# getzlab/rnaseqc

Hardware: AMD Instinct MI355X
Metric: reads/sec whole-node (100 M-read synthetic BAM, GENCODE GTF) at 1/2/4/8 GPU -- `value`: the hot path over the records resident in HBM (the bench contract's definition of value); `whole_node.value`: the same job from the BAM file to the reports (CLI `Average Reads/Sec` window), checked against `value (higher is better)
Workload: dtype i32/u64 counters, f64 exon fractions

## Files before the change

rnaseqc_amd/csrc/rsqc_api.cpp:

```cpp
#include "rsqc_ctx.h"
#include "rsqc_index.h"

namespace rsqc {

int fail(rsqc_ctx *c, int code, const std::string &msg) {
    if (c) { c->last_error = msg; }
    return code;
}
int dev_alloc(rsqc_ctx *c, DevBuf &b, size_t bytes, bool zero) {
    if (bytes == 0) bytes = 16;
    bytes = (bytes + 15) & ~(size_t)15;
    if (b.bytes < bytes) {
        b.release();
        HIP_TRY(c, hipMalloc(&b.p, bytes));
        b.bytes = bytes;
    }
    if (zero) HIP_TRY(c, hipMemsetAsync(b.p, 0, b.bytes, c->stream));
    return 0;
}
bool dev_reserve(DevBuf &b, size_t bytes) {
    if (b.bytes >= bytes) return true;
    b.release();
    if (hipMalloc(&b.p, bytes) != hipSuccess) { (void)hipGetLastError(); b.p = nullptr; return false; }
    b.bytes = bytes;
    return true;
}
bool host_reserve(HostBuf &b, size_t bytes) {
    if (b.bytes >= bytes) return true;
    b.release();
    if (hipHostMalloc(&b.p, bytes, hipHostMallocDefault) != hipSuccess) { (void)hipGetLastError(); b.p = nullptr; return false; }
    b.bytes = bytes;
    return true;
}

static int zero_accumulators(rsqc_ctx *c) {
    launch_reset(c->stream, c->d_arena.p, c->arena_bytes, c->d_cov.p, c->d_cov.bytes, (uint32_t *)((char *)c->d_arena.p + c->off_misc + 36));
    HIP_TRY(c, hipGetLastError());
    for (auto &pb : c->pair_pool) pb.used = false;
    c->pairs_in_flight.clear();
    c->pair_arena.used = c->frag_arena.used = c->gc_arena.used = 0;
    for (auto &fb : c->frag_pool) fb.used = false;
    c->frags_in_flight.clear();
    c->h_fsize.clear(); c->h_fcount.clear();
    c->frag_remaining = c->have_bed ? c->params.fragment_samples : 0;
    for (auto &gb : c->gc_pool) gb.used = false;
    c->gcs_in_flight.clear();
    if (c->have_ref) {
        HIP_TRY(c, hipMemsetAsync(c->d_gc_bins.p, 0, (RSQC_GC_BINS + 1) * 8, c->stream));
        c->h_gc.assign(RSQC_GC_BINS + 1, 0);
    }
    c->finalized = false;
    c->next_record_base = 0; c->name_mode = -1; c->have_ranges = false; c->have_composed_rl = false;
    c->batch_file_index.clear(); c->batch_records.clear();
    c->h_rl_offset.clear(); c->h_rl_span.clear(); c->h_rl_state.clear();
    c->h_sample_file.clear(); c->h_sample_size.clear(); c->frag_kept = 0;
    c->sticky = 0;
    return 0;
}

// ... 57 lines not shown
        if (D.ev_copy) (void)hipEventDestroy(D.ev_copy);
        if (D.copy_stream) (void)hipStreamDestroy(D.copy_stream);
        for (auto &e : D.pe) if (e) (void)hipEventDestroy(e);
    }
    sort_drop(c);
    markdup_drop(c);
    junction_drop(c, true);
    track_drop(c, true);
    genebody_drop(c, true);
    tin_drop(c, true);
    cycle_drop(c, true);
    mismatch_drop(c, true);
    for (auto &b : c->parked) b.release();
    free_sort_scratch(c->gc_scratch); free_sort_scratch(c->frag_scratch);
    c->d_ref_bits.release(); c->d_ref_off.release(); c->d_ref_len.release(); c->d_gc_bins.release(); c->d_exon_gc.release();
    DevBuf *all[] = {&c->d_arena, &c->d_cov, &c->d_ovf_index, &c->d_tiles, &c->d_defer, &c->d_ei_rank, &c->d_table, &c->d_tab_off, &c->d_tab_cap};
    if (c->h_arena) (void)hipHostFree(c->h_arena);
    if (c->h_rl_raw) (void)hipHostFree(c->h_rl_raw);
    if (c->stream2) (void)hipStreamDestroy(c->stream2);
    if (c->stream3) (void)hipStreamDestroy(c->stream3);
    if (c->stream4) (void)hipStreamDestroy(c->stream4);
    if (c->ev_join3) (void)hipEventDestroy(c->ev_join3);
    if (c->ev_join4) (void)hipEventDestroy(c->ev_join4);
    if (c->ev_fork) (void)hipEventDestroy(c->ev_fork);
    if (c->ev_retired) (void)hipEventDestroy(c->ev_retired);
    if (c->ev_join) (void)hipEventDestroy(c->ev_join);
    for (auto *b : all) b->release();
    for (auto &pr : c->k1_events) { (void)hipEventDestroy(pr.first); (void)hipEventDestroy(pr.second); }
    for (auto &pr : c->long_events) (void)hipEventDestroy(pr.second);
    for (auto e : c->event_pool) (void)hipEventDestroy(e);
    (void)hipStreamDestroy(c->stream);
    delete c;
}

int rsqc_set_annotation(rsqc_ctx *c, const rsqc_annotation *a, const uint8_t *owned_contig) {
    if (!c || !a) return RSQC_ERR_ARG;
    if (c->have_ann) return fail(c, RSQC_ERR_ARG, "annotation already set");
    HIP_TRY(c, hipSetDevice(c->device));
    const int nc = a->n_contigs, G = a->n_genes, L = a->n_genes_listed, E = a->n_exons;
    c->n_ref = a->n_ref; c->n_contigs = nc; c->n_genes = G; c->n_listed = L; c->n_exons = E;
    HostIndex hx;
    {
        std::string err;
        int brc = hx.build(a, owned_contig, err);
        if (brc) return fail(c, brc, err);
    }
    const uint64_t run = hx.cov_entries;
// ... 47 lines not shown
#undef UPV
#undef UPA
    const size_t n_u64 = (size_t)G * 3 + RSQC_N_COUNTERS;
    const size_t Lz = (size_t)std::max(L, 1), Ez = (size_t)std::max(E, 1);
    auto pad8 = [](size_t x) { return (x + 7) & ~(size_t)7; };
    size_t at = 0;
    c->off_u64 = at; at += n_u64 * 8;
    c->off_bias3 = at; at += Lz * 8;
    c->off_bias5 = at; at += Lz * 8;
    c->off_exon = at; at += Ez * 8;
    c->off_gmean = at; at += Lz * 8;
    c->off_gstd = at; at += Lz * 8;
    c->off_gcv = at; at += Lz * 8;
    c->off_ecv = at; at += Ez * 8;
    c->off_gvalid = at; at += pad8(Lz);
    c->off_ecvv = at; at += pad8(Ez);
    c->off_ehit = at; at += pad8(Ez);
    at = (at + 15) & ~(size_t)15;
    c->off_misc = at; at += 64;
    c->arena_bytes = at;
    if ((rc = dev_alloc(c, c->d_arena, at, false))) return rc;
    HIP_TRY(c, hipHostMalloc((void **)&c->h_arena, at, hipHostMallocDefault));
    if ((rc = dev_alloc(c, c->d_cov, (size_t)(run + 64) * 4, false))) return rc;
    const uint32_t ovf_cap = 1u << 20;
    if ((rc = dev_alloc(c, c->d_ovf_index, (size_t)ovf_cap * 8, false))) return rc;
    for (hipStream_t *s : {&c->stream2, &c->stream3, &c->stream4})
        if (!*s) HIP_TRY(c, hipStreamCreateWithPriority(s, hipStreamNonBlocking, c->prio_side));
    for (hipEvent_t *e : {&c->ev_join3, &c->ev_join4, &c->ev_fork, &c->ev_join, &c->ev_retired})
        if (!*e) HIP_TRY(c, hipEventCreateWithFlags(e, hipEventDisableTiming));
    char *A = (char *)c->d_arena.p;
    DevAccum &acc = c->acc;
    acc.gene_reads = (unsigned long long *)(A + c->off_u64);
    acc.gene_unique = acc.gene_reads + G;
    acc.gene_frag = acc.gene_unique + G;
    acc.counters = acc.gene_frag + G;
    acc.exon_acc = (double *)(A + c->off_exon);
    acc.cov_diff = (uint32_t *)c->d_cov.p;
    acc.ovf_count = (uint32_t *)(A + c->off_misc);
    acc.read_length = (int32_t *)(A + c->off_misc + 8);
    acc.error = (int *)(A + c->off_misc + 16);
    acc.rl_stats = (uint32_t *)(A + c->off_misc + 32);
    acc.defer_total = (uint32_t *)(A + c->off_misc + 48);
    acc.ovf_index = (uint64_t *)c->d_ovf_index.p; acc.ovf_cap = ovf_cap;
    c->have_ann = true;
    if ((rc = zero_accumulators(c))) return rc;
    HIP_TRY(c, hipStreamSynchronize(c->stream));
    c->last_error = hx.warning;
    c->n_exons_outside_gene = hx.n_exons_outside_gene;
    return RSQC_OK;
}

// ... 126 lines not shown
    for (auto &pb : c->pair_pool) pb.used = false;
    for (auto &fb : c->frag_pool) fb.used = false;
    for (auto &gb : c->gc_pool) gb.used = false;
    c->pairs_in_flight.clear(); c->frags_in_flight.clear(); c->gcs_in_flight.clear();
    for (Arena *a : {&c->pair_arena, &c->frag_arena, &c->gc_arena}) {
        for (int k = 0; k < a->n_col; ++k) a->col[k].release();
        a->used = a->cap = 0;
    }
    for (auto &b : c->ann_bufs) b.release();
    c->ann_bufs.clear();
    for (DevBuf *b : {&c->d_arena, &c->d_cov, &c->d_ei_rank, &c->d_ovf_index, &c->d_table, &c->d_tab_off, &c->d_tab_cap,
                      &c->d_ref_bits, &c->d_ref_off, &c->d_ref_len, &c->d_gc_bins, &c->d_exon_gc,
                      &c->d_rl_summary}) b->release();
    if (c->h_arena) { (void)hipHostFree(c->h_arena); c->h_arena = nullptr; }
    c->arena_bytes = 0;
    c->dann = DevAnnotation{}; c->dref = DevReference{};
    uint32_t *const tile_span = c->acc.tile_span;
    c->acc = DevAccum{}; c->acc.tile_span = tile_span;
    c->d_ge_off = c->d_ge_row = c->d_gene_cov_off = c->d_gene_coding = c->d_gene_order = nullptr;
    c->d_gene_flags = c->d_gene_owned = nullptr;
    c->n_ref = c->n_contigs = c->n_genes = c->n_listed = c->n_exons = 0;
    c->k3_large = c->k3_medium = c->k3_xlarge = c->k3_le6144 = c->k3_le3072 = c->k3_le2048 = c->k3_le1024 = 0;
    c->cov_entries = 0; c->n_exons_outside_gene = 0;
    std::vector<uint32_t>().swap(c->exon_row_id);
    std::vector<double>().swap(c->h_exon_gc);
    c->h_gc.clear();
    c->have_ann = c->have_bed = c->have_ref = false;
    free_sort_scratch(c->gc_scratch); free_sort_scratch(c->frag_scratch);
    c->h_fsize.clear(); c->h_fcount.clear(); c->frag_remaining = 0; c->frag_kept = 0;
    c->finalized = false; c->early_copied = false;
    c->next_record_base = 0; c->name_mode = -1; c->have_ranges = false; c->have_composed_rl = false;
    c->batch_file_index.clear(); c->batch_records.clear();
    c->h_rl_offset.clear(); c->h_rl_span.clear(); c->h_rl_state.clear();
    c->h_sample_file.clear(); c->h_sample_size.clear();
    c->results = rsqc_results{};
    c->sticky = 0;
    c->last_error.clear();
    return RSQC_OK;
}

void *rsqc_host_alloc(size_t bytes) {
    void *p = nullptr;
    if (hipHostMalloc(&p, bytes ? bytes : 16, hipHostMallocDefault) != hipSuccess) { (void)hipGetLastError(); return nullptr; }
    return p;
}
void rsqc_host_free(void *p) { if (p) (void)hipHostFree(p); }
// ... 49 lines not shown
```

rnaseqc_amd/csrc/rsqc_ctx.h:

```cpp
#pragma once
#include <algorithm>
#include <chrono>
#include <cstdio>
#include <cstdlib>
#include <cstring>
#include <string>
#include <vector>

#include "rsqc_device.h"
#include "rsqc_decode.h"
#include "rsqc_sam.h"

#if defined(RSQC_K1_PROF) || defined(RSQC_DIAG_KNOBS)
#define RSQC_DIAG(name) getenv(name)
namespace rsqc {
inline void host_trace(const char *what) {
    static const bool on = getenv("RSQC_HOST_TRACE") != nullptr;
    if (!on) return;
    static std::chrono::steady_clock::time_point last = std::chrono::steady_clock::now();
    const auto now = std::chrono::steady_clock::now();
    fprintf(stderr, "[host] %-28s +%8.1f us\n", what, std::chrono::duration<double, std::micro>(now - last).count());
    last = now;
}
}
// ... 192 lines not shown
    bool have_ann = false;
    int32_t n_ref = 0, n_contigs = 0, n_genes = 0, n_listed = 0, n_exons = 0;
    std::vector<uint32_t> exon_row_id;
    std::vector<DevBuf> ann_bufs;
    DevAnnotation dann{};
    DevParams dparams{};
    const uint32_t *d_ge_off = nullptr, *d_ge_row = nullptr, *d_gene_cov_off = nullptr, *d_gene_coding = nullptr;
    const uint8_t *d_gene_flags = nullptr, *d_gene_owned = nullptr;
    const uint32_t *d_gene_order = nullptr;
    uint32_t k3_large = 0, k3_medium = 0, k3_xlarge = 0, k3_le6144 = 0, k3_le3072 = 0, k3_le2048 = 0, k3_le1024 = 0;
    int stream_prio = 0, prio_side = 0;
    uint32_t n_exons_outside_gene = 0;
    hipEvent_t fin_e0 = nullptr, fin_e1 = nullptr;
    uint64_t cov_entries = 0;
    bool have_bed = false;

    DevBuf d_arena, d_cov, d_ovf_index, d_tiles;
    DevBuf d_defer;
    DevBuf d_ei_rank;
    char *h_arena = nullptr;
    size_t arena_bytes = 0, off_u64 = 0, off_exon = 0, off_gmean = 0, off_gstd = 0, off_gcv = 0, off_bias3 = 0,
           off_bias5 = 0, off_ecv = 0, off_gvalid = 0, off_ecvv = 0, off_ehit = 0, off_misc = 0;
    hipStream_t stream2 = nullptr, stream3 = nullptr, stream4 = nullptr;
    hipEvent_t ev_fork = nullptr, ev_join = nullptr, ev_join3 = nullptr, ev_join4 = nullptr, ev_retired = nullptr;
    DevAccum acc{};
    uint64_t tile_cap = 0;
    std::vector<PairBuf> pair_pool;
    std::vector<size_t> pairs_in_flight;
    Arena pair_arena, frag_arena, gc_arena;
    DevBuf d_arena_count;
    std::vector<DevBuf> parked;
    DevBuf d_table, d_tab_off, d_tab_cap;
    std::vector<FragBuf> frag_pool;
    std::vector<size_t> frags_in_flight;
    uint32_t frag_remaining = 0;
    bool have_ref = false;
    DevBuf d_ref_bits, d_ref_off, d_ref_len, d_gc_bins, d_exon_gc;
    DevReference dref{};
    std::vector<GcBuf> gc_pool;
    std::vector<size_t> gcs_in_flight;
    std::vector<uint64_t> h_gc;
    std::vector<double> h_exon_gc;
    SortScratch gc_scratch, frag_scratch;
    uint32_t frag_kept = 0;
    bool finalized = false;

    std::vector<UploadedBatch *> resident;
// ... 110 lines not shown
```

rnaseqc_amd/csrc/rsqc_device.h:

```cpp
#pragma once

#if !defined(RSQC_WAVE_EMU)
#include <hip/hip_runtime.h>
#endif
#include <stdint.h>

#include "rsqc_read.h"

#define RSQC_K1_THREADS 256
#define RSQC_MAX_BIAS_WINDOW 1024
#define RSQC_K3_THREADS 1024
#include "rsqc_k3_plan.h"

namespace rsqc {

struct DevBatch {
    uint64_t n;
    uint64_t record_base;
    const rsqc_rec_core *core;
    const rsqc_rec_aux *aux;
    const uint32_t *cigar;
    const uint32_t *qhash2;
    uint32_t n_seg;
    const int32_t *seg_tid;
// ... 79 lines not shown
    const uint32_t *ex_cov;
    const uint32_t *ex_id;
    const uint32_t *gene_cov_off;
    const uint32_t *gene_coding;
    const uint8_t *gene_flags;
    const uint8_t *gene_owned;
    const uint32_t *gene_order;
    const unsigned long long *gene_reads;
    uint32_t *cov;
    int32_t n_listed;
    uint32_t mask; int32_t bias_offset, bias_window; uint64_t bias_gene_length;
    double *g_mean, *g_std, *g_cv; uint8_t *g_valid;
    double *e_cv; uint8_t *e_cv_valid;
    unsigned long long *bias3, *bias5;
    int *error;
};
void launch_gene_coverage(hipStream_t s, hipStream_t s2, hipStream_t s3, const GeneCovArgs &A, uint32_t n_large, uint32_t n_medium, uint32_t n_xlarge,
                          uint32_t n_le6144 = 0, uint32_t n_le3072 = 0, uint32_t n_le2048 = 0, uint32_t n_le1024 = 0);

void launch_reduce_add(hipStream_t s, unsigned long long *du, const unsigned long long *su, size_t nu, double *df, const double *sf, size_t nf,
                       uint8_t *db, const uint8_t *sb, size_t nb);
void launch_pack_results(hipStream_t s, const double *exon_acc, uint8_t *exon_hit, uint32_t n_exons);
void launch_reset(hipStream_t s, void *arena, size_t arena_bytes, void *cov, size_t cov_bytes, uint32_t *rl_min);
void launch_classify(hipStream_t s, int grid, int variant, const DevAnnotation &a, const DevParams &p, const DevBatch &b,
                     const DevAccum &acc);
inline int rsqc_long_grid(int k1_grid) { return k1_grid < 1024 ? k1_grid : 1024; }
void launch_classify_long(hipStream_t s, int k1_grid, const DevAnnotation &a, const DevParams &p, const DevBatch &b, const DevAccum &acc);
void launch_ei_rank(hipStream_t s, const EiEntry *ei, uint32_t ei_lo, uint32_t ei_hi, EiRank *rank, uint32_t n_words);
void launch_classify_slow(hipStream_t s, const DevAnnotation &a, const DevParams &p, const DevBatch &b,
                          const DevAccum &acc);
#define RSQC_RL_SUMMARY_WORDS (2 + 2 * 128)
void launch_read_length(hipStream_t s, const DevAnnotation &a, const DevParams &p, const DevBatch &b,
                        const DevAccum &acc, uint32_t *summary);
#define RSQC_SLOW_RES 2048u
#define RSQC_SLOW_LEGACY_GRID 4096u
#ifndef RSQC_K4_PART_READS
#define RSQC_K4_PART_READS 1024
#endif
#define RSQC_K4_SUB_CAP (2 * RSQC_K4_PART_READS)
#define RSQC_K4_PART_SLOTS (4 * RSQC_K4_PART_READS)
#ifndef RSQC_K4_COUNT_THREADS
#define RSQC_K4_COUNT_THREADS 256
#endif
struct FragKey { uint32_t lo, hi, h2; };
struct FragPlan {
    uint32_t *part_first;
// ... 30 lines not shown
```

rnaseqc_amd/csrc/rsqc_finalize.cpp:

```cpp
#include "rsqc_ctx.h"
#include "rsqc_rl_compose.h"

static int read_back(rsqc_ctx *c) {
    const int G = c->n_genes, L = c->n_listed, E = c->n_exons;
    char *A = (char *)c->d_arena.p;
    if (c->early_copied) {
        const size_t frag_lo = c->off_u64 + (size_t)2 * (size_t)G * 8;
        HIP_TRY(c, hipMemcpyAsync(c->h_arena + frag_lo, (char *)c->d_arena.p + frag_lo, (size_t)G * 8, hipMemcpyDeviceToHost, c->stream));
        HIP_TRY(c, hipMemcpyAsync(c->h_arena + c->off_misc, (char *)c->d_arena.p + c->off_misc, c->arena_bytes - c->off_misc, hipMemcpyDeviceToHost, c->stream));
        c->early_copied = false;
        RSQC_TRACE("read_back: copies enqueued");
    } else {
        launch_pack_results(c->stream, (const double *)(A + c->off_exon), (uint8_t *)(A + c->off_ehit), (uint32_t)E);
        HIP_TRY(c, hipMemcpyAsync(c->h_arena, c->d_arena.p, c->arena_bytes, hipMemcpyDeviceToHost, c->stream));
    }
    HIP_TRY(c, hipStreamSynchronize(c->stream));
    RSQC_TRACE("read_back: stream idle");
    char *H = c->h_arena;
    uint64_t *u = (uint64_t *)(H + c->off_u64);
    rsqc_results &R = c->results;
    for (int k = 0; k < RSQC_N_COUNTERS; ++k) R.counters[k] = u[3 * (size_t)G + (size_t)k];
    R.n_genes_listed = L; R.n_exons = E;
    R.gene_reads = u; R.gene_unique = u + G; R.gene_fragments = u + 2 * (size_t)G;
    R.exon_reads = (double *)(H + c->off_exon); R.exon_hit = (uint8_t *)(H + c->off_ehit);
// ... 1 lines not shown
    R.gene_cov_mean = (double *)(H + c->off_gmean); R.gene_cov_std = (double *)(H + c->off_gstd); R.gene_cov_cv = (double *)(H + c->off_gcv);
    R.gene_cov_valid = (uint8_t *)(H + c->off_gvalid); R.exon_cv = (double *)(H + c->off_ecv); R.exon_cv_valid = (uint8_t *)(H + c->off_ecvv);
    R.bias_three = (uint64_t *)(H + c->off_bias3); R.bias_five = (uint64_t *)(H + c->off_bias5);
    R.n_fragment_sizes = (uint32_t)c->h_fsize.size();
    R.fragment_size = c->h_fsize.data(); R.fragment_count = c->h_fcount.data();
    R.fragment_samples_remaining = c->frag_remaining;
    R.have_reference = c->have_ref ? 1 : 0;
    R.gc_bins = c->have_ref ? c->h_gc.data() : nullptr;
    R.gc_out_of_range = c->have_ref ? c->h_gc[RSQC_GC_BINS] : 0;
    R.exon_gc = c->have_ref ? c->h_exon_gc.data() : nullptr;
    R.exons_outside_gene_row = c->n_exons_outside_gene;
    c->timing.slow_records = *(const uint32_t *)(H + c->off_misc + 4);
    const int err = *(const int *)(H + c->off_misc + 16);
    if (err) {
        c->sticky = err;
        return fail(c, err, device_error_message(c, err));
    }
    return 0;
}

static int run_finalize_kernels(rsqc_ctx *c, bool early_readback = false) {
    int rc;
    c->early_copied = false;
    const int G = c->n_genes, L = c->n_listed;
    char *A = (char *)c->d_arena.p;
    hipEvent_t e0 = get_event(c), e1 = get_event(c);
        HIP_TRY(c, hipEventRecord(e0, c->stream));
        HIP_TRY(c, hipEventRecord(c->ev_fork, c->stream));
        HIP_TRY(c, hipStreamWaitEvent(c->stream2, c->ev_fork, 0));
        HIP_TRY(c, hipStreamWaitEvent(c->stream3, c->ev_fork, 0));
        HIP_TRY(c, hipStreamWaitEvent(c->stream4, c->ev_fork, 0));
        GeneCovArgs Ga{};
        Ga.ge_off = c->d_ge_off; Ga.ge_row = c->d_ge_row;
        Ga.ex = c->dann.ex; Ga.ex_cov = c->dann.ex_cov; Ga.ex_id = c->dann.ex_id;
        Ga.gene_cov_off = c->d_gene_cov_off; Ga.gene_coding = c->d_gene_coding;
        Ga.gene_flags = c->d_gene_flags; Ga.gene_owned = c->d_gene_owned;
        Ga.gene_order = c->d_gene_order;
        Ga.gene_reads = c->acc.gene_reads; Ga.cov = c->acc.cov_diff; Ga.n_listed = L;
        Ga.mask = c->params.coverage_mask; Ga.bias_offset = c->params.bias_offset; Ga.bias_window = c->params.bias_window;
        Ga.bias_gene_length = c->params.bias_gene_length;
        Ga.g_mean = (double *)(A + c->off_gmean); Ga.g_std = (double *)(A + c->off_gstd); Ga.g_cv = (double *)(A + c->off_gcv);
        Ga.g_valid = (uint8_t *)(A + c->off_gvalid); Ga.e_cv = (double *)(A + c->off_ecv); Ga.e_cv_valid = (uint8_t *)(A + c->off_ecvv);
        Ga.bias3 = (unsigned long long *)(A + c->off_bias3); Ga.bias5 = (unsigned long long *)(A + c->off_bias5);
        Ga.error = c->acc.error;
        {
            uint32_t nl = c->k3_large, nm = c->k3_medium, nx = c->k3_xlarge;
            if (const char *e = RSQC_DIAG("RSQC_K3_FORCE")) {
                const int f = atoi(e);
                if (f == 1) { nl = (uint32_t)L; nm = 0; } else if (f == 2) { nl = 0; nm = (uint32_t)L; nx = 0; } else if (f == 3) { nl = 0; nm = 0; nx = 0; } else if (f == 4) { nl = (uint32_t)L; nm = 0; nx = (uint32_t)L; }
            }
            if (!RSQC_DIAG("RSQC_DIAG_SKIP_K3")) launch_gene_coverage(c->stream2, c->stream3, c->stream4, Ga, nl, nm, nx, c->k3_le6144, c->k3_le3072, c->k3_le2048, c->k3_le1024);
        }
        bool retired_here = false;
        if (c->pairs_in_flight.size() > 1) {
// ... 37 lines not shown
                acc.pairs = (PairRec *)pb.rec.p;
                acc.pair_chunk_cap = pb.chunk_cap; acc.pair_chunk_count = (uint32_t *)pb.counts.p;
                acc.pair_slow_base = pb.slow_base; acc.pair_slow_cap = pb.slow_cap;
                acc.pair_slow_count = (uint32_t *)pb.counts.p + pb.n_chunks;
                launch_frag_local(c->stream, acc, pb.n_chunks, P, c->dparams.legacy ? (uint32_t)std::min<uint64_t>(4096, pb.slow_cap / 8192 + 32) : 0u);
            }
            if (!RSQC_DIAG("RSQC_DIAG_SKIP_K4")) launch_frag_count(c->stream, (uint32_t)G, P, (uint32_t)parts_bound, c->acc.gene_frag, c->acc.error);
        }
        RSQC_TRACE("finalize: K3 + K4 enqueued");
        {
            const size_t nb = c->batch_file_index.size();
            if (nb * RSQC_RL_SUMMARY_WORDS > c->h_rl_raw_cap) {
                if (c->h_rl_raw) { (void)hipHostFree(c->h_rl_raw); c->h_rl_raw = nullptr; c->h_rl_raw_cap = 0; }
                const size_t want = std::max<size_t>(2 * nb, 64) * RSQC_RL_SUMMARY_WORDS;
                HIP_TRY(c, hipHostMalloc((void **)&c->h_rl_raw, want * 4, hipHostMallocDefault));
                c->h_rl_raw_cap = want;
            }
            RSQC_TRACE("finalize: K3 enqueued");
            if (nb) HIP_TRY(c, hipMemcpyAsync(c->h_rl_raw, c->d_rl_summary.p, nb * RSQC_RL_SUMMARY_WORDS * 4, hipMemcpyDeviceToHost, c->stream2));
            RSQC_TRACE("finalize: rl copy call returned");
        }
        HIP_TRY(c, hipEventRecord(c->ev_join3, c->stream3));
        HIP_TRY(c, hipEventRecord(c->ev_join4, c->stream4));
        if (early_readback) {
            const size_t frag_lo = c->off_u64 + (size_t)2 * (size_t)c->n_genes * 8, frag_hi = frag_lo + (size_t)c->n_genes * 8;
            HIP_TRY(c, hipStreamWaitEvent(c->stream2, c->ev_join3, 0));
            HIP_TRY(c, hipStreamWaitEvent(c->stream2, c->ev_join4, 0));
            launch_pack_results(c->stream2, (const double *)(A + c->off_exon), (uint8_t *)(A + c->off_ehit), (uint32_t)c->n_exons);
            if (frag_lo) HIP_TRY(c, hipMemcpyAsync(c->h_arena, c->d_arena.p, frag_lo, hipMemcpyDeviceToHost, c->stream2));
            HIP_TRY(c, hipMemcpyAsync(c->h_arena + frag_hi, (char *)c->d_arena.p + frag_hi, c->off_misc - frag_hi, hipMemcpyDeviceToHost, c->stream2));
            c->early_copied = true;
        }
        HIP_TRY(c, hipEventRecord(c->ev_join, c->stream2));
        HIP_TRY(c, hipStreamWaitEvent(c->stream, c->ev_join, 0));
        HIP_TRY(c, hipStreamWaitEvent(c->stream, c->ev_join3, 0));
        HIP_TRY(c, hipStreamWaitEvent(c->stream, c->ev_join4, 0));
        HIP_TRY(c, hipGetLastError());
        HIP_TRY(c, hipEventRecord(e1, c->stream));
        if (c->have_bed) {
            uint64_t incoming = 0;
            bool beside = true;
#ifdef RSQC_K5_SERIAL
            beside = false;
#endif
            HIP_TRY(c, hipEventSynchronize(c->ev_fork));
            for (size_t k = 0; k < c->frags_in_flight.size(); ++k) incoming += *c->frag_pool[c->frags_in_flight[k]].h_count;
            if (c->frag_arena.used && c->frag_arena.used + incoming > c->frag_arena.cap) beside = false;
            hipStream_t ks = beside ? c->stream4 : c->stream;
            if (!beside) HIP_TRY(c, hipStreamSynchronize(c->stream));
            else if (retired_here) HIP_TRY(c, hipStreamWaitEvent(ks, c->ev_retired, 0));
            for (size_t k = 0; k < c->frags_in_flight.size(); ++k) {
                FragBuf &fb = c->frag_pool[c->frags_in_flight[k]];
                const uint32_t n = *fb.h_count;
                if (n > fb.cap) return fail(c, RSQC_ERR_CAPACITY, "fragment candidate overflow");
                const void *src[6] = {fb.file.p, fb.qhash.p, fb.name.p, fb.endpos.p, fb.fs.p, fb.h2.p};
                if ((rc = arena_append(c, c->frag_arena, src, n, ks))) return rc;
                fb.used = false;
            }
            c->frags_in_flight.clear();
            const uint64_t total = c->frag_arena.used;
            if (total > 0xFFFFFFF0ull) return fail(c, RSQC_ERR_CAPACITY, "too many fragment-size candidates");
            FragCandidates fc{(uint64_t *)c->frag_arena.col[0].p, (uint64_t *)c->frag_arena.col[1].p, (int32_t *)c->frag_arena.col[2].p,
                              (int32_t *)c->frag_arena.col[3].p, (uint32_t *)c->frag_arena.col[4].p, nullptr, (uint32_t)total, nullptr, (uint32_t *)c->frag_arena.col[5].p};
            const auto tf0 = std::chrono::steady_clock::now();
            rc = run_fragment_sizes(ks, fc, (uint32_t)total, c->params.fragment_samples, c->h_fsize, c->h_fcount,
                                    c->frag_remaining, c->frag_scratch, c->frag_kept, c->acc.error);
            if (beside && !rc) HIP_TRY(c, hipStreamSynchronize(ks));
            c->timing.fragment_sizes_ms += std::chrono::duration<double, std::milli>(std::chrono::steady_clock::now() - tf0).count();
// ... 41 lines not shown
        const uint32_t *w = c->h_rl_raw + k * RSQC_RL_SUMMARY_WORDS;
        const uint32_t P = std::min<uint32_t>(w[0], 128u);
        for (uint32_t j = 0; j < P; ++j) { c->h_rl_span.push_back(w[2 + 2 * j]); c->h_rl_state.push_back((int32_t)w[3 + 2 * j]); }
        c->h_rl_offset[k + 1] = (uint32_t)c->h_rl_span.size();
    }
}
static int32_t compose_read_length(const rsqc_ctx *c) {
    std::vector<rsqc::RlTable> tables(c->batch_file_index.size());
    for (size_t k = 0; k < tables.size(); ++k)
        tables[k] = rsqc::RlTable{c->batch_file_index[k], c->h_rl_span.data() + c->h_rl_offset[k], c->h_rl_state.data() + c->h_rl_offset[k],
                                  c->h_rl_offset[k + 1] - c->h_rl_offset[k]};
    return rsqc::rl_compose(tables);
}
static void finish_finalize_bookkeeping(rsqc_ctx *c) {
    float ms = 0.f;
    if (c->fin_e0 && hipEventElapsedTime(&ms, c->fin_e0, c->fin_e1) == hipSuccess) c->timing.finalize_ms += ms;
    if (c->fin_e0) { c->event_pool.push_back(c->fin_e0); c->event_pool.push_back(c->fin_e1); c->fin_e0 = c->fin_e1 = nullptr; }
    resolve_events(c);
    for (auto *u : c->transient) retire_batch(c, u);
    c->transient.clear();
    unpack_rl_summaries(c);
    if (c->have_ranges) { c->composed_rl = compose_read_length(c); c->have_composed_rl = true; c->results.read_length = c->composed_rl; }
    free_parked(c);
    c->finalized = true;
}

int rsqc_finalize(rsqc_ctx *c, rsqc_results *out) {
    if (!c || !out || !c->have_ann) return RSQC_ERR_ARG;
    if (c->sticky) return c->sticky;
    if (c->sort.active) return fail(c, RSQC_ERR_ARG, "rsqc_sort_end must precede rsqc_finalize (a collection of rsqc_sort_begin is open)");
    HIP_TRY(c, hipSetDevice(c->device));
    int rc;
    if (!c->finalized) {
        RSQC_TRACE("finalize: enter");
        if ((rc = run_finalize_kernels(c, true))) return rc;
        RSQC_TRACE("finalize: kernels enqueued");
        if ((rc = read_back(c))) return rc;
        finish_finalize_bookkeeping(c);
        RSQC_TRACE("finalize: bookkeeping done");
    } else if ((rc = read_back(c))) return rc;
    *out = c->results;
    return RSQC_OK;
}

int rsqc_finalize_device(rsqc_ctx *c) {
    if (!c || !c->have_ann) return RSQC_ERR_ARG;
// ... 70 lines not shown
```

rnaseqc_amd/csrc/rsqc_k4.h:

```cpp
#pragma once

namespace rsqc {


__device__ __forceinline__ uint32_t frag_part_hash(uint64_t key) {
    uint32_t h = (uint32_t)(key >> 32);
    h ^= h >> 15; h *= 0x2C1B3C6Du; h ^= h >> 12;
    return h;
}
__device__ __forceinline__ uint32_t frag_parts_of(unsigned long long reads) {
    return (uint32_t)((reads + RSQC_K4_PART_READS - 1) / RSQC_K4_PART_READS);
}
__device__ __forceinline__ uint32_t frag_cap_of(unsigned long long reads) {
    return frag_parts_of(reads) == 1 ? (uint32_t)reads : (uint32_t)RSQC_K4_SUB_CAP;
}
__device__ __forceinline__ unsigned long long frag_space_of(unsigned long long reads) {
    return ((unsigned long long)frag_parts_of(reads) * frag_cap_of(reads) + 15ull) & ~15ull;
}
__global__ void __launch_bounds__(1024)
frag_layout_totals_kernel(const unsigned long long *gene_reads, uint32_t n_genes, unsigned long long *blk_space, uint32_t *blk_parts, int *error) {
    __shared__ unsigned long long w_space[16];
    __shared__ uint32_t w_parts[16];
    const uint32_t g = blockIdx.x * 1024u + threadIdx.x;
    unsigned long long space = 0; uint32_t parts = 0;
    if (g < n_genes) {
        const unsigned long long n = gene_reads[g];
        if (n > 0xFFFFFFF0ull) atomicExch(error, RSQC_ERR_CAPACITY);
        parts = frag_parts_of(n); space = frag_space_of(n);
    }
    space = wave_sum(space); parts = wave_sum(parts);
    if (lane_id() == 0) { w_space[threadIdx.x >> 6] = space; w_parts[threadIdx.x >> 6] = parts; }
    __syncthreads();
    if (threadIdx.x == 0) {
        unsigned long long s = 0; uint32_t p = 0;
        for (int w = 0; w < 16; ++w) { s += w_space[w]; p += w_parts[w]; }
        blk_space[blockIdx.x] = s; blk_parts[blockIdx.x] = p;
    }
}
__global__ void __launch_bounds__(1024)
frag_layout_kernel(const unsigned long long *gene_reads, uint32_t n_genes, const unsigned long long *blk_space, const uint32_t *blk_parts,
                   uint32_t *part_first, uint4 *ginfo, uint32_t *cursor, uint4 *part_info, uint32_t *full_n) {
    __shared__ unsigned long long w_space[16];
    __shared__ uint32_t w_parts[16];
    __shared__ unsigned long long s_base; __shared__ uint32_t p_base;
    const int l = lane_id(), wv = (int)(threadIdx.x >> 6);
    if (wv == 0) {
        unsigned long long s = 0; uint32_t p = 0;
        for (uint32_t k = (uint32_t)l; k < blockIdx.x; k += 64) { s += blk_space[k]; p += blk_parts[k]; }
        s = wave_sum(s); p = wave_sum(p);
        if (l == 0) { s_base = s; p_base = p; }
    }
    const uint32_t g = blockIdx.x * 1024u + threadIdx.x;
    unsigned long long space = 0; uint32_t parts = 0, cap = 0;
    if (g < n_genes) { const unsigned long long n = gene_reads[g]; parts = frag_parts_of(n); cap = frag_cap_of(n); space = frag_space_of(n); }
    unsigned long long isp = space; uint32_t ipt = parts;
#pragma unroll
    for (int o = 1; o < 64; o <<= 1) {
        const unsigned long long ts = __shfl_up(isp, o, 64); const uint32_t tp = __shfl_up(ipt, o, 64);
        if (l >= o) { isp += ts; ipt += tp; }
    }
    if (l == 63) { w_space[wv] = isp; w_parts[wv] = ipt; }
    __syncthreads();
    unsigned long long bs = s_base; uint32_t bp = p_base;
    for (int w = 0; w < wv; ++w) { bs += w_space[w]; bp += w_parts[w]; }
    const uint32_t pf = bp + ipt - parts; const unsigned long long gb = bs + isp - space;
    if (g < n_genes) { part_first[g] = pf; ginfo[g] = make_uint4(pf, parts, cap, (uint32_t)(gb >> 4)); }
    if (g == n_genes - 1) part_first[n_genes] = bp + ipt;
    if (g == 0) *full_n = 0u;
    if (parts >= 1) { cursor[pf] = 0u; part_info[pf] = make_uint4(g, cap, (uint32_t)gb, (uint32_t)(gb >> 32)); }
    unsigned long long big = __ballot(parts > 1);
    while (big) {
        const int src = __ffsll(big) - 1; big &= big - 1;
        const uint32_t pf_s = lane_value(pf, src), n_s = lane_value(parts, src), cap_s = lane_value(cap, src), g_s = lane_value(g, src);
        const unsigned long long gb_s = (unsigned long long)lane_value((uint32_t)gb, src) | ((unsigned long long)lane_value((uint32_t)(gb >> 32), src) << 32);
        for (uint32_t k = 1u + (uint32_t)l; k < n_s; k += 64) {
            const unsigned long long off = gb_s + (unsigned long long)k * cap_s;
            cursor[pf_s + k] = 0u; part_info[pf_s + k] = make_uint4(g_s, cap_s, (uint32_t)off, (uint32_t)(off >> 32));
        }
    }
}

#ifndef RSQC_K4L_THREADS
#define RSQC_K4L_THREADS 512
#endif
#ifndef RSQC_K4L_U
#define RSQC_K4L_U 4
#endif
#define RSQC_K4L_PIECE (RSQC_K4L_U * RSQC_K4L_THREADS)
#define RSQC_K4L_GSLOTS RSQC_K4L_PIECE
constexpr int k4l_log2(unsigned v) { return v <= 1 ? 0 : 1 + k4l_log2(v >> 1); }
#ifndef RSQC_K4L_WIN
#define RSQC_K4L_WIN 2048
#endif
#ifndef RSQC_K4L_CHUNKS
#define RSQC_K4L_CHUNKS 2
#endif
inline uint32_t frag_local_chunk_wgs(uint32_t n_chunks) { return (n_chunks + RSQC_K4L_CHUNKS - 1u) / RSQC_K4L_CHUNKS; }
struct K4LocalShared {
    uint32_t gkey[RSQC_K4L_GSLOTS], gcnt[RSQC_K4L_GSLOTS];
    unsigned long long win[RSQC_K4L_WIN];
    uint32_t win2[RSQC_K4L_WIN];
};
// ... 270 lines not shown
```

rnaseqc_amd/csrc/rsqc_kernels.hip:

```cpp
#include <hip/hip_runtime.h>
#include <stdint.h>
#include <algorithm>
#include <cstdlib>

#ifdef RSQC_K1_PROF
namespace rsqc { __device__ __forceinline__ void k1_mark(int sec); __device__ __forceinline__ void k1_event(int id, bool cond); }
#define RSQC_MARK(sec) ::rsqc::k1_mark(sec)
#define RSQC_EVENT(id, cond) ::rsqc::k1_event(id, cond)
#endif

#include "rsqc_device.h"
#ifndef RSQC_K1_PROF
#define RSQC_FIN_STAMP(sec)
#define RSQC_FIN_SECT(base, sec)
#define RSQC_FIN_BEGIN
#endif

namespace rsqc {

}
#include "rsqc_wave.h"
namespace rsqc {

#ifdef RSQC_K1_PROF
// ... 270 lines not shown
    for (size_t i = (size_t)blockIdx.x * blockDim.x + threadIdx.x; i < arena_vec; i += stride) arena[i] = i == rl_vec ? armed : z;
}

__global__ void __launch_bounds__(256)
reduce_add_kernel(unsigned long long *du, const unsigned long long *su, size_t nu, double *df, const double *sf, size_t nf,
                  uint8_t *db, const uint8_t *sb, size_t nb) {
    const size_t stride = (size_t)gridDim.x * blockDim.x, t = (size_t)blockIdx.x * blockDim.x + threadIdx.x;
    for (size_t i = t; i < nu; i += stride) du[i] += su[i];
    for (size_t i = t; i < nf; i += stride) df[i] += sf[i];
    for (size_t i = t; i < nb; i += stride) db[i] = (uint8_t)(db[i] + sb[i]);
}
void launch_reduce_add(hipStream_t s, unsigned long long *du, const unsigned long long *su, size_t nu, double *df, const double *sf, size_t nf,
                       uint8_t *db, const uint8_t *sb, size_t nb) {
    hipLaunchKernelGGL(reduce_add_kernel, dim3(512), dim3(256), 0, s, du, su, nu, df, sf, nf, db, sb, nb);
}

void launch_pack_results(hipStream_t s, const double *exon_acc, uint8_t *exon_hit, uint32_t n_exons) {
    if (n_exons) hipLaunchKernelGGL(pack_results_kernel, dim3((n_exons + 255) / 256 < 1024 ? (n_exons + 255) / 256 : 1024), dim3(256), 0, s, exon_acc, exon_hit, n_exons);
}
void launch_reset(hipStream_t s, void *arena, size_t arena_bytes, void *cov, size_t cov_bytes, uint32_t *rl_min) {
    const size_t rl_vec = (size_t)((char *)rl_min - 4 - (char *)arena) / 16;
    hipLaunchKernelGGL(reset_kernel, dim3(1024), dim3(256), 0, s, (uint4 *)arena, (arena_bytes + 15) / 16, (uint4 *)cov, (cov_bytes + 15) / 16, rl_vec);
}
void launch_frag_compact(hipStream_t s, const FragCandidates &src, const FragCandidates &dst, uint64_t n_rec, int k1_grid) {
    hipLaunchKernelGGL(frag_compact_kernel, dim3(k1_grid), dim3(256), 0, s, src, dst, (uint32_t)n_rec, (uint32_t)k1_grid);
}
void launch_classify(hipStream_t s, int grid, int variant, const DevAnnotation &a, const DevParams &p, const DevBatch &b,
                     const DevAccum &acc) {
    if (variant < 0) hipLaunchKernelGGL(classify_count_kernel_legacy, dim3(grid), dim3(RSQC_K1_THREADS), 0, s, a, p, b, acc);
    else {
#if defined(RSQC_K1_PROF) || defined(RSQC_DIAG_KNOBS)
        static const unsigned pad = getenv("RSQC_K1_LDS_PAD") ? (unsigned)atoi(getenv("RSQC_K1_LDS_PAD")) : 0u;
#else
        const unsigned pad = 0u;
#endif
        const K1Args A{a, p, b, acc};
        if (a.have_bed) hipLaunchKernelGGL(classify_ei_kernel<true>, dim3(grid), dim3(RSQC_K1_THREADS), pad, s, A);
        else hipLaunchKernelGGL(classify_ei_kernel<false>, dim3(grid), dim3(RSQC_K1_THREADS), pad, s, A);
    }
}
void launch_classify_long(hipStream_t s, int k1_grid, const DevAnnotation &a, const DevParams &p, const DevBatch &b, const DevAccum &acc) {
    const K1Args A{a, p, b, acc};
    hipLaunchKernelGGL(classify_long_kernel, dim3((unsigned)rsqc_long_grid(k1_grid)), dim3(RSQC_K1_THREADS), 0, s, A, (uint32_t)k1_grid);
}
void launch_classify_slow(hipStream_t s, const DevAnnotation &a, const DevParams &p, const DevBatch &b,
                          const DevAccum &acc) {
    if (p.legacy) {
        const uint64_t blocks = (b.n + RSQC_SLOW_THREADS - 1) / RSQC_SLOW_THREADS;
        hipLaunchKernelGGL(classify_slow_kernel<true>, dim3((unsigned)std::min<uint64_t>(blocks ? blocks : 1, RSQC_SLOW_LEGACY_GRID)), dim3(RSQC_SLOW_THREADS), 0, s, a, p, b, acc);
    } else {
        const uint64_t blocks = std::max<uint64_t>(64, std::min<uint64_t>(2048, b.n / 200 / RSQC_SLOW_THREADS + 1));
        hipLaunchKernelGGL(classify_slow_kernel<false>, dim3((unsigned)blocks), dim3(RSQC_SLOW_THREADS), 0, s, a, p, b, acc);
    }
}
void launch_read_length(hipStream_t s, const DevAnnotation &a, const DevParams &p, const DevBatch &b,
                        const DevAccum &acc, uint32_t *summary) {
    hipLaunchKernelGGL(read_length_kernel, dim3(acc.rl_seg ? b.n_seg : 1u), dim3(64), 0, s, a, p, b, acc, summary);
}
void launch_frag_layout(hipStream_t s, const unsigned long long *gene_reads, uint32_t n_genes, const FragPlan &P, int *error) {
    const uint32_t blocks = (n_genes + 1023u) / 1024u;
    if (!blocks) return;
    hipLaunchKernelGGL(frag_layout_totals_kernel, dim3(blocks), dim3(1024), 0, s, gene_reads, n_genes, P.blk_space, P.blk_parts, error);
    hipLaunchKernelGGL(frag_layout_kernel, dim3(blocks), dim3(1024), 0, s, gene_reads, n_genes, P.blk_space, P.blk_parts, P.part_first,
                       P.ginfo, P.cursor, P.part_info, P.full_n);
}
void launch_frag_local(hipStream_t s, const DevAccum &acc, uint32_t n_chunks, const FragPlan &P, uint32_t list_blocks) {
    hipLaunchKernelGGL(frag_local_kernel, dim3(frag_local_chunk_wgs(n_chunks) + (list_blocks ? list_blocks : RSQC_K4_SLOW_BLOCKS)), dim3(RSQC_K4L_THREADS), 0, s, acc.pairs, acc.pair_chunk_cap, acc.pair_chunk_count, n_chunks, acc.pair_slow_base, acc.pair_slow_cap,
                       P.ginfo, P.cursor, P.list, acc.error);
}
void launch_frag_count(hipStream_t s, uint32_t n_genes, const FragPlan &P, uint32_t parts_bound, unsigned long long *gene_frag, int *error) {
    if (n_genes == 0) return;
    const uint32_t grid = parts_bound < 16384u ? (parts_bound ? parts_bound : 1u) : 16384u;
    hipLaunchKernelGGL((frag_count_kernel<RSQC_K4_PART_SLOTS / 2>), dim3(grid), dim3(RSQC_K4_COUNT_THREADS), 0, s, P.part_first + n_genes, P.cursor, P.part_info, P.list, gene_frag,
                       P.full_list, P.full_n, error);
    hipLaunchKernelGGL((frag_count_kernel<RSQC_K4_PART_SLOTS>), dim3(grid < 1024u ? grid : 1024u), dim3(RSQC_K4_COUNT_THREADS), 0, s, P.part_first + n_genes, P.cursor, P.part_info, P.list, gene_frag,
                       P.full_list, P.full_n, error);
}
#ifndef RSQC_K3_MEDIUM_T
#define RSQC_K3_MEDIUM_T uint32_t
#endif
#ifndef RSQC_K3_SMALL_T
#define RSQC_K3_SMALL_T uint32_t
#endif
void launch_gene_coverage(hipStream_t s, hipStream_t s2, hipStream_t s3, const GeneCovArgs &A, uint32_t n_large, uint32_t n_medium, uint32_t n_xlarge,
                          uint32_t n_le6144, uint32_t n_le3072, uint32_t n_le2048, uint32_t n_le1024) {
    if (A.n_listed <= 0) return;
    K3Launch plan[RSQC_K3_LAUNCHES];
// ... 28 lines not shown
```

Before: 26.60 billion.

## Clear coverage buffer on side stream during finalize and fuse frag layout kernels

Result: no change. 26.71 billion (median of 4 runs) (+0.4%).

```diff
diff --git a/rnaseqc_amd/csrc/rsqc_api.cpp b/rnaseqc_amd/csrc/rsqc_api.cpp
--- a/rnaseqc_amd/csrc/rsqc_api.cpp
+++ b/rnaseqc_amd/csrc/rsqc_api.cpp
@@ -34,7 +34,10 @@
 }
 
 static int zero_accumulators(rsqc_ctx *c) {
-    launch_reset(c->stream, c->d_arena.p, c->arena_bytes, c->d_cov.p, c->d_cov.bytes, (uint32_t *)((char *)c->d_arena.p + c->off_misc + 36));
+    const bool cov_is_zero = c->cov_clean && c->finalized && !c->sticky;
+    if (c->cov_clear_enqueued && !cov_is_zero) HIP_TRY(c, hipStreamWaitEvent(c->stream, c->ev_join, 0));
+    launch_reset(c->stream, c->d_arena.p, c->arena_bytes, c->d_cov.p, cov_is_zero ? 0 : c->d_cov.bytes, (uint32_t *)((char *)c->d_arena.p + c->off_misc + 36));
+    c->cov_clean = c->cov_clear_enqueued = false;
     HIP_TRY(c, hipGetLastError());
     for (auto &pb : c->pair_pool) pb.used = false;
     c->pairs_in_flight.clear();
@@ -138,7 +141,6 @@
     if (c->stream4) (void)hipStreamDestroy(c->stream4);
     if (c->ev_join3) (void)hipEventDestroy(c->ev_join3);
     if (c->ev_join4) (void)hipEventDestroy(c->ev_join4);
-    if (c->ev_fork) (void)hipEventDestroy(c->ev_fork);
     if (c->ev_retired) (void)hipEventDestroy(c->ev_retired);
     if (c->ev_join) (void)hipEventDestroy(c->ev_join);
     for (auto *b : all) b->release();
@@ -232,11 +234,12 @@
     if ((rc = dev_alloc(c, c->d_arena, at, false))) return rc;
     HIP_TRY(c, hipHostMalloc((void **)&c->h_arena, at, hipHostMallocDefault));
     if ((rc = dev_alloc(c, c->d_cov, (size_t)(run + 64) * 4, false))) return rc;
+    c->cov_clean = c->cov_clear_enqueued = false;
     const uint32_t ovf_cap = 1u << 20;
     if ((rc = dev_alloc(c, c->d_ovf_index, (size_t)ovf_cap * 8, false))) return rc;
     for (hipStream_t *s : {&c->stream2, &c->stream3, &c->stream4})
         if (!*s) HIP_TRY(c, hipStreamCreateWithPriority(s, hipStreamNonBlocking, c->prio_side));
-    for (hipEvent_t *e : {&c->ev_join3, &c->ev_join4, &c->ev_fork, &c->ev_join, &c->ev_retired})
+    for (hipEvent_t *e : {&c->ev_join3, &c->ev_join4, &c->ev_join, &c->ev_retired})
         if (!*e) HIP_TRY(c, hipEventCreateWithFlags(e, hipEventDisableTiming));
     char *A = (char *)c->d_arena.p;
     DevAccum &acc = c->acc;
@@ -409,6 +412,7 @@
     c->n_ref = c->n_contigs = c->n_genes = c->n_listed = c->n_exons = 0;
     c->k3_large = c->k3_medium = c->k3_xlarge = c->k3_le6144 = c->k3_le3072 = c->k3_le2048 = c->k3_le1024 = 0;
     c->cov_entries = 0; c->n_exons_outside_gene = 0;
+    c->cov_clean = c->cov_clear_enqueued = false;
     std::vector<uint32_t>().swap(c->exon_row_id);
     std::vector<double>().swap(c->h_exon_gc);
     c->h_gc.clear();
diff --git a/rnaseqc_amd/csrc/rsqc_ctx.h b/rnaseqc_amd/csrc/rsqc_ctx.h
--- a/rnaseqc_amd/csrc/rsqc_ctx.h
+++ b/rnaseqc_amd/csrc/rsqc_ctx.h
@@ -238,7 +238,8 @@
     size_t arena_bytes = 0, off_u64 = 0, off_exon = 0, off_gmean = 0, off_gstd = 0, off_gcv = 0, off_bias3 = 0,
            off_bias5 = 0, off_ecv = 0, off_gvalid = 0, off_ecvv = 0, off_ehit = 0, off_misc = 0;
     hipStream_t stream2 = nullptr, stream3 = nullptr, stream4 = nullptr;
-    hipEvent_t ev_fork = nullptr, ev_join = nullptr, ev_join3 = nullptr, ev_join4 = nullptr, ev_retired = nullptr;
+    hipEvent_t ev_join = nullptr, ev_join3 = nullptr, ev_join4 = nullptr, ev_retired = nullptr;
+    bool cov_clear_enqueued = false, cov_clean = false;
     DevAccum acc{};
     uint64_t tile_cap = 0;
     std::vector<PairBuf> pair_pool;
diff --git a/rnaseqc_amd/csrc/rsqc_device.h b/rnaseqc_amd/csrc/rsqc_device.h
--- a/rnaseqc_amd/csrc/rsqc_device.h
+++ b/rnaseqc_amd/csrc/rsqc_device.h
@@ -125,6 +125,7 @@
                        uint8_t *db, const uint8_t *sb, size_t nb);
 void launch_pack_results(hipStream_t s, const double *exon_acc, uint8_t *exon_hit, uint32_t n_exons);
 void launch_reset(hipStream_t s, void *arena, size_t arena_bytes, void *cov, size_t cov_bytes, uint32_t *rl_min);
+void launch_clear_cov(hipStream_t s, void *cov, size_t cov_bytes);
 void launch_classify(hipStream_t s, int grid, int variant, const DevAnnotation &a, const DevParams &p, const DevBatch &b,
                      const DevAccum &acc);
 inline int rsqc_long_grid(int k1_grid) { return k1_grid < 1024 ? k1_grid : 1024; }
diff --git a/rnaseqc_amd/csrc/rsqc_finalize.cpp b/rnaseqc_amd/csrc/rsqc_finalize.cpp
--- a/rnaseqc_amd/csrc/rsqc_finalize.cpp
+++ b/rnaseqc_amd/csrc/rsqc_finalize.cpp
@@ -47,14 +47,14 @@
 static int run_finalize_kernels(rsqc_ctx *c, bool early_readback = false) {
     int rc;
     c->early_copied = false;
+    c->cov_clean = false;
     const int G = c->n_genes, L = c->n_listed;
     char *A = (char *)c->d_arena.p;
     hipEvent_t e0 = get_event(c), e1 = get_event(c);
         HIP_TRY(c, hipEventRecord(e0, c->stream));
-        HIP_TRY(c, hipEventRecord(c->ev_fork, c->stream));
-        HIP_TRY(c, hipStreamWaitEvent(c->stream2, c->ev_fork, 0));
-        HIP_TRY(c, hipStreamWaitEvent(c->stream3, c->ev_fork, 0));
-        HIP_TRY(c, hipStreamWaitEvent(c->stream4, c->ev_fork, 0));
+        HIP_TRY(c, hipStreamWaitEvent(c->stream2, e0, 0));
+        HIP_TRY(c, hipStreamWaitEvent(c->stream3, e0, 0));
+        HIP_TRY(c, hipStreamWaitEvent(c->stream4, e0, 0));
         GeneCovArgs Ga{};
         Ga.ge_off = c->d_ge_off; Ga.ge_row = c->d_ge_row;
         Ga.ex = c->dann.ex; Ga.ex_cov = c->dann.ex_cov; Ga.ex_id = c->dann.ex_id;
@@ -138,19 +138,19 @@
         }
         HIP_TRY(c, hipEventRecord(c->ev_join3, c->stream3));
         HIP_TRY(c, hipEventRecord(c->ev_join4, c->stream4));
+        HIP_TRY(c, hipStreamWaitEvent(c->stream2, c->ev_join3, 0));
+        HIP_TRY(c, hipStreamWaitEvent(c->stream2, c->ev_join4, 0));
         if (early_readback) {
             const size_t frag_lo = c->off_u64 + (size_t)2 * (size_t)c->n_genes * 8, frag_hi = frag_lo + (size_t)c->n_genes * 8;
-            HIP_TRY(c, hipStreamWaitEvent(c->stream2, c->ev_join3, 0));
-            HIP_TRY(c, hipStreamWaitEvent(c->stream2, c->ev_join4, 0));
             launch_pack_results(c->stream2, (const double *)(A + c->off_exon), (uint8_t *)(A + c->off_ehit), (uint32_t)c->n_exons);
             if (frag_lo) HIP_TRY(c, hipMemcpyAsync(c->h_arena, c->d_arena.p, frag_lo, hipMemcpyDeviceToHost, c->stream2));
             HIP_TRY(c, hipMemcpyAsync(c->h_arena + frag_hi, (char *)c->d_arena.p + frag_hi, c->off_misc - frag_hi, hipMemcpyDeviceToHost, c->stream2));
             c->early_copied = true;
         }
+        launch_clear_cov(c->stream2, c->d_cov.p, c->d_cov.bytes);
+        c->cov_clear_enqueued = true;
         HIP_TRY(c, hipEventRecord(c->ev_join, c->stream2));
         HIP_TRY(c, hipStreamWaitEvent(c->stream, c->ev_join, 0));
-        HIP_TRY(c, hipStreamWaitEvent(c->stream, c->ev_join3, 0));
-        HIP_TRY(c, hipStreamWaitEvent(c->stream, c->ev_join4, 0));
         HIP_TRY(c, hipGetLastError());
         HIP_TRY(c, hipEventRecord(e1, c->stream));
         if (c->have_bed) {
@@ -159,7 +159,7 @@
 #ifdef RSQC_K5_SERIAL
             beside = false;
 #endif
-            HIP_TRY(c, hipEventSynchronize(c->ev_fork));
+            HIP_TRY(c, hipEventSynchronize(e0));
             for (size_t k = 0; k < c->frags_in_flight.size(); ++k) incoming += *c->frag_pool[c->frags_in_flight[k]].h_count;
             if (c->frag_arena.used && c->frag_arena.used + incoming > c->frag_arena.cap) beside = false;
             hipStream_t ks = beside ? c->stream4 : c->stream;
@@ -247,6 +247,7 @@
     unpack_rl_summaries(c);
     if (c->have_ranges) { c->composed_rl = compose_read_length(c); c->have_composed_rl = true; c->results.read_length = c->composed_rl; }
     free_parked(c);
+    c->cov_clean = c->cov_clear_enqueued;
     c->finalized = true;
 }
 
diff --git a/rnaseqc_amd/csrc/rsqc_k4.h b/rnaseqc_amd/csrc/rsqc_k4.h
--- a/rnaseqc_amd/csrc/rsqc_k4.h
+++ b/rnaseqc_amd/csrc/rsqc_k4.h
@@ -37,19 +37,10 @@
         blk_space[blockIdx.x] = s; blk_parts[blockIdx.x] = p;
     }
 }
-__global__ void __launch_bounds__(1024)
-frag_layout_kernel(const unsigned long long *gene_reads, uint32_t n_genes, const unsigned long long *blk_space, const uint32_t *blk_parts,
-                   uint32_t *part_first, uint4 *ginfo, uint32_t *cursor, uint4 *part_info, uint32_t *full_n) {
-    __shared__ unsigned long long w_space[16];
-    __shared__ uint32_t w_parts[16];
-    __shared__ unsigned long long s_base; __shared__ uint32_t p_base;
+__device__ __forceinline__ void frag_layout_rows(const unsigned long long *gene_reads, uint32_t n_genes, unsigned long long (&w_space)[16], uint32_t (&w_parts)[16],
+                                                 const unsigned long long &s_base, const uint32_t &p_base,
+                                                 uint32_t *part_first, uint4 *ginfo, uint32_t *cursor, uint4 *part_info, uint32_t *full_n) {
     const int l = lane_id(), wv = (int)(threadIdx.x >> 6);
-    if (wv == 0) {
-        unsigned long long s = 0; uint32_t p = 0;
-        for (uint32_t k = (uint32_t)l; k < blockIdx.x; k += 64) { s += blk_space[k]; p += blk_parts[k]; }
-        s = wave_sum(s); p = wave_sum(p);
-        if (l == 0) { s_base = s; p_base = p; }
-    }
     const uint32_t g = blockIdx.x * 1024u + threadIdx.x;
     unsigned long long space = 0; uint32_t parts = 0, cap = 0;
     if (g < n_genes) { const unsigned long long n = gene_reads[g]; parts = frag_parts_of(n); cap = frag_cap_of(n); space = frag_space_of(n); }
@@ -78,6 +69,52 @@
             cursor[pf_s + k] = 0u; part_info[pf_s + k] = make_uint4(g_s, cap_s, (uint32_t)off, (uint32_t)(off >> 32));
         }
     }
+}
+__global__ void __launch_bounds__(1024)
+frag_layout_kernel(const unsigned long long *gene_reads, uint32_t n_genes, const unsigned long long *blk_space, const uint32_t *blk_parts,
+                   uint32_t *part_first, uint4 *ginfo, uint32_t *cursor, uint4 *part_info, uint32_t *full_n) {
+    __shared__ unsigned long long w_space[16];
+    __shared__ uint32_t w_parts[16];
+    __shared__ unsigned long long s_base; __shared__ uint32_t p_base;
+    const int l = lane_id(), wv = (int)(threadIdx.x >> 6);
+    if (wv == 0) {
+        unsigned long long s = 0; uint32_t p = 0;
+        for (uint32_t k = (uint32_t)l; k < blockIdx.x; k += 64) { s += blk_space[k]; p += blk_parts[k]; }
+        s = wave_sum(s); p = wave_sum(p);
+        if (l == 0) { s_base = s; p_base = p; }
+    }
+    frag_layout_rows(gene_reads, n_genes, w_space, w_parts, s_base, p_base, part_first, ginfo, cursor, part_info, full_n);
+}
+__global__ void __launch_bounds__(1024)
+frag_layout_fused_kernel(const unsigned long long *gene_reads, uint32_t n_genes, uint32_t *part_first, uint4 *ginfo, uint32_t *cursor,
+                         uint4 *part_info, uint32_t *full_n, int *error) {
+    __shared__ unsigned long long w_space[16];
+    __shared__ uint32_t w_parts[16];
+    __shared__ unsigned long long f_space[16];
+    __shared__ uint32_t f_parts[16];
+    __shared__ unsigned long long s_base; __shared__ uint32_t p_base;
+    const int l = lane_id(), wv = (int)(threadIdx.x >> 6);
+    {
+        const uint32_t g_own = blockIdx.x * 1024u + threadIdx.x, front = blockIdx.x * 1024u;
+        if (g_own < n_genes && gene_reads[g_own] > 0xFFFFFFF0ull) atomicExch(error, RSQC_ERR_CAPACITY);
+        unsigned long long s = 0; uint32_t p = 0;
+        for (uint32_t k0 = threadIdx.x; k0 < front; k0 += 16u * 1024u) {
+            unsigned long long n[16];
+#pragma unroll
+            for (int j = 0; j < 16; ++j) { const uint32_t k = k0 + (uint32_t)j * 1024u; n[j] = k < front ? gene_reads[k] : 0ull; }
+#pragma unroll
+            for (int j = 0; j < 16; ++j) { s += frag_space_of(n[j]); p += frag_parts_of(n[j]); }
+        }
+        s = wave_sum(s); p = wave_sum(p);
+        if (l == 0) { f_space[wv] = s; f_parts[wv] = p; }
+        __syncthreads();
+        if (threadIdx.x == 0) {
+            unsigned long long ts = 0; uint32_t tp = 0;
+            for (int w = 0; w < 16; ++w) { ts += f_space[w]; tp += f_parts[w]; }
+            s_base = ts; p_base = tp;
+        }
+    }
+    frag_layout_rows(gene_reads, n_genes, w_space, w_parts, s_base, p_base, part_first, ginfo, cursor, part_info, full_n);
 }
 
 #ifndef RSQC_K4L_THREADS
diff --git a/rnaseqc_amd/csrc/rsqc_kernels.hip b/rnaseqc_amd/csrc/rsqc_kernels.hip
--- a/rnaseqc_amd/csrc/rsqc_kernels.hip
+++ b/rnaseqc_amd/csrc/rsqc_kernels.hip
@@ -316,6 +316,9 @@
     const size_t rl_vec = (size_t)((char *)rl_min - 4 - (char *)arena) / 16;
     hipLaunchKernelGGL(reset_kernel, dim3(1024), dim3(256), 0, s, (uint4 *)arena, (arena_bytes + 15) / 16, (uint4 *)cov, (cov_bytes + 15) / 16, rl_vec);
 }
+void launch_clear_cov(hipStream_t s, void *cov, size_t cov_bytes) {
+    hipLaunchKernelGGL(reset_kernel, dim3(1024), dim3(256), 0, s, (uint4 *)nullptr, (size_t)0, (uint4 *)cov, (cov_bytes + 15) / 16, (size_t)0);
+}
 void launch_frag_compact(hipStream_t s, const FragCandidates &src, const FragCandidates &dst, uint64_t n_rec, int k1_grid) {
     hipLaunchKernelGGL(frag_compact_kernel, dim3(k1_grid), dim3(256), 0, s, src, dst, (uint32_t)n_rec, (uint32_t)k1_grid);
 }
@@ -354,9 +357,7 @@
 void launch_frag_layout(hipStream_t s, const unsigned long long *gene_reads, uint32_t n_genes, const FragPlan &P, int *error) {
     const uint32_t blocks = (n_genes + 1023u) / 1024u;
     if (!blocks) return;
-    hipLaunchKernelGGL(frag_layout_totals_kernel, dim3(blocks), dim3(1024), 0, s, gene_reads, n_genes, P.blk_space, P.blk_parts, error);
-    hipLaunchKernelGGL(frag_layout_kernel, dim3(blocks), dim3(1024), 0, s, gene_reads, n_genes, P.blk_space, P.blk_parts, P.part_first,
-                       P.ginfo, P.cursor, P.part_info, P.full_n);
+    hipLaunchKernelGGL(frag_layout_fused_kernel, dim3(blocks), dim3(1024), 0, s, gene_reads, n_genes, P.part_first, P.ginfo, P.cursor, P.part_info, P.full_n, error);
 }
 void launch_frag_local(hipStream_t s, const DevAccum &acc, uint32_t n_chunks, const FragPlan &P, uint32_t list_blocks) {
     hipLaunchKernelGGL(frag_local_kernel, dim3(frag_local_chunk_wgs(n_chunks) + (list_blocks ? list_blocks : RSQC_K4_SLOW_BLOCKS)), dim3(RSQC_K4L_THREADS), 0, s, acc.pairs, acc.pair_chunk_cap, acc.pair_chunk_count, n_chunks, acc.pair_slow_base, acc.pair_slow_cap,
```
